# returaj/gan_mpc

Hardware: AMD Instinct MI355X
Metric: trajectories/sec (rollout+backward+critic step) at batch=1024, H=50 (higher is better)
Workload: dtype f32

## Files before the change

### gan_mpc_amd/csrc/gmpc_traj_rw.hip

```cpp
#include "gmpc_traj_layers.h"
#include "gmpc_ls_common.h"
#include "gmpc_launch.h"

#define GMPC_RW_THREADS 256
__host__ __device__ constexpr int rw_xk(int KH, int NHL) { return KH * NHL > 320 ? 64 : 0; }
__host__ __device__ constexpr int rw_khp(int KH) { return KH + 4; }
__host__ __device__ constexpr int rw_kb(int KH, int w) {
  return KH == 200 ? (w == 0 ? 0 : w == 1 ? 52 : w == 2 ? 104 : w == 3 ? 152 : 200) : (KH / 4) * w;
}

__host__ __device__ constexpr bool rw_row_in_lds(int k, int QX) { return (k >> 3) < QX && (k & 2) != 0; }
__host__ __device__ constexpr int rw_reg_index(int k, int QX) {
  int r = 0;
  for (int j = 0; j < k; ++j) r += rw_row_in_lds(j, QX) ? 0 : 1;
  return r;
}

__device__ __forceinline__ void rw_hidden_epilogue(f32x4_t d, int nn, int H, float4* hout, uint32_t* mbase,
                                                   size_t mstride, unsigned wbits) {
  const int lane = threadIdx.x & 63, wave = threadIdx.x >> 6;
  const bool valid = nn < H;
  const bool on0 = d[0] > 0.f && valid, on1 = d[1] > 0.f && valid;
  const bool on2 = d[2] > 0.f && valid, on3 = d[3] > 0.f && valid;
  const unsigned long long w0 = __ballot(on0), w1 = __ballot(on1), w2 = __ballot(on2), w3 = __ballot(on3);
  if (mbase != nullptr) {
    const unsigned long long word = lane == 0 ? w0 : lane == 1 ? w1 : lane == 2 ? w2 : w3;
    if (lane < 4 && ((wbits >> lane) & 1u)) {
      uint32_t* mp = mbase + (size_t)lane * mstride + 2 * wave;
      mp[0] = (uint32_t)word;
      mp[1] = (uint32_t)(word >> 32);
    }
  }
  if (valid) hout[nn] = make_float4(on0 ? d[0] : 0.f, on1 ? d[1] : 0.f, on2 ? d[2] : 0.f, on3 ? d[3] : 0.f);
}

template <int H, int XK>
__device__ __forceinline__ f32x4_t rw_layer(const float* wr, const float4* hin, const float4* wx, float bias) {
  static_assert(H % 8 == 0 && XK % 4 == 0 && 2 * XK <= H, "H");
  const int lane = threadIdx.x & 63;
  const float* hf = reinterpret_cast<const float*>(hin);
  constexpr int NR = (4 * H + 63) / 64;
  constexpr int QX = XK / 4;
  float ar[NR];
#pragma unroll
  for (int r = 0; r < NR; ++r) ar[r] = hf[64 * r + lane];
  constexpr int DX = 3;
  float4 xq[DX];
#pragma unroll
  for (int j = 0; j < DX; ++j)
    xq[j] = j < QX ? wx[j * GMPC_RW_THREADS + threadIdx.x] : make_float4(0.f, 0.f, 0.f, 0.f);
  f32x4_t d0 = {bias, bias, bias, bias}, d1 = {0.f, 0.f, 0.f, 0.f};
  __builtin_amdgcn_sched_barrier(0);
  rw_static_for<H / 8>([&](auto qc) __attribute__((always_inline)) {
    constexpr int q = decltype(qc)::value;
    const float4 x = xq[q % DX];
    if (q < QX && q + DX < QX) xq[q % DX] = wx[(q + DX) * GMPC_RW_THREADS + threadIdx.x];
    rw_static_for<8>([&](auto ec) __attribute__((always_inline)) {
      constexpr int e = decltype(ec)::value;
      constexpr int k = 8 * q + e;
      float w;
      if constexpr (rw_row_in_lds(k, QX)) w = e == 2 ? x.x : e == 3 ? x.y : e == 6 ? x.z : x.w;
      else { constexpr int ri = rw_reg_index(k, QX); w = wr[ri]; }
      if constexpr (e & 1) rw_mfma<k>(d1, ar[k >> 4], w);
      else rw_mfma<k>(d0, ar[k >> 4], w);
    });
    __builtin_amdgcn_sched_group_barrier(0x100, 1, 0);
    __builtin_amdgcn_sched_group_barrier(0x008, 8, 0);
  });
  return d0 + d1;
}

template <int K0, int K1, int KHP>
__device__ __forceinline__ f32x4_t rw_out_part(const float4* hin, const float* wlT, int n) {
  static_assert(K0 % 4 == 0 && K1 % 4 == 0 && K1 > K0, "float4 reads of the weight row");
  const int lane = threadIdx.x & 63;
  const float* hf = reinterpret_cast<const float*>(hin);
  constexpr int R0 = K0 >> 4, R1 = (K1 - 1) >> 4;
  float ar[R1 - R0 + 1];
#pragma unroll
  for (int r = R0; r <= R1; ++r) ar[r - R0] = hf[64 * r + lane];
  const float4* wrow = reinterpret_cast<const float4*>(wlT + (size_t)(lane < n ? lane : n - 1) * KHP + K0);
  float4 wv[(K1 - K0) / 4];
#pragma unroll
  for (int q = 0; q < (K1 - K0) / 4; ++q) wv[q] = wrow[q];
  f32x4_t d0 = {0.f, 0.f, 0.f, 0.f}, d1 = {0.f, 0.f, 0.f, 0.f};
  __builtin_amdgcn_sched_barrier(0);
  rw_static_for<(K1 - K0) / 4>([&](auto qc) __attribute__((always_inline)) {
    constexpr int q = decltype(qc)::value;
    constexpr int k = K0 + 4 * q;
    rw_mfma<k + 0>(d0, ar[((k + 0) >> 4) - R0], wv[q].x);
    rw_mfma<k + 1>(d1, ar[((k + 1) >> 4) - R0], wv[q].y);
    rw_mfma<k + 2>(d0, ar[((k + 2) >> 4) - R0], wv[q].z);
    rw_mfma<k + 3>(d1, ar[((k + 3) >> 4) - R0], wv[q].w);
  });
  return d0 + d1;
}

template <bool LS, int KH, int NHL, int K0Q>
__global__ __launch_bounds__(GMPC_RW_THREADS, 1) void k_traj_rw(TrajArgs a) {
  static_assert(KH % 16 == 0 || KH == 200, "output-layer K split in multiples of 4");
  constexpr int XK = rw_xk(KH, NHL), KHP = rw_khp(KH);
  extern __shared__ __attribute__((aligned(16))) char smem_traj[];
  float4* const actA = reinterpret_cast<float4*>(smem_traj);
  float4* const actB = actA + a.aw;
  float4* const part = actB + a.aw;
  float4* const ksp = part + a.pw;
  float4* const xcur = ksp + GMPC_THREADS;
  float* const wl_s = reinterpret_cast<float*>(xcur + 32);
  float4* const wx_s = reinterpret_cast<float4*>(wl_s + a.swl);
  __shared__ float s_alpha[GMPC_TB];
  __shared__ int s_bi[GMPC_TB], s_in[GMPC_TB];

  const int tid = threadIdx.x, wave = tid >> 6, lane = tid & 63;
  const int n = a.n, m = a.m, T = a.T;
  const int b0 = blockIdx.x * GMPC_TB;
  if (LS) {
    const int cnt = *a.nitems;
    if (b0 >= cnt || ls_round_form(cnt, a) != LS_FORM_RW) return;
    if (tid < GMPC_TB) ls_candidate(a, cnt, b0 + tid, &s_bi[tid], &s_in[tid], &s_alpha[tid]);
  } else if (tid < GMPC_TB) {
    s_bi[tid] = min(b0 + tid, a.B - 1);
    s_in[tid] = (b0 + tid) < a.B;
  }
  __syncthreads();
  float* const xf = reinterpret_cast<float*>(xcur);
  float* const aAf = reinterpret_cast<float*>(actA);
  const float* const pf = reinterpret_cast<const float*>(part);
  auto BI = [&](int c) -> int { return s_bi[c]; };
  auto INB = [&](int c) -> bool { return s_in[c] != 0; };
  auto CI = [&](int c) -> size_t { return (size_t)(b0 + c); };
  const int Lh = a.dyn.L - 1;
  const size_t mstride = (size_t)T * Lh * GMPC_MW;
  for (int e = tid; e < n * KHP; e += blockDim.x) {
    const int no = e / KHP, k = e - no * KHP;
    wl_s[e] = k < KH ? a.dyn.W[Lh][(size_t)k * n + no] : 0.f;
  }
  const float w0 = sigmoidf_(a.mpc_w[0]), w1 = sigmoidf_(a.mpc_w[1]), w2 = sigmoidf_(a.mpc_w[2]);

  const int nnA = 64 * wave + lane;
  float wr[NHL][KH];
  float w0r[4 * K0Q];
  float rbias[NHL + 1];
  {
#pragma unroll
    for (int k = 0; k < 4 * K0Q; ++k)
      w0r[k] = (k < n + m && nnA < KH) ? a.dyn.W[0][(size_t)k * KH + nnA] : 0.f;
    rw_static_for<NHL>([&](auto hc) __attribute__((always_inline)) {
      constexpr int hl = decltype(hc)::value;
      const float* Wl = a.dyn.W[hl + 1];
      constexpr int qx = hl == NHL - 1 ? XK / 4 : 0;
      rw_static_for<KH>([&](auto kc) __attribute__((always_inline)) {
        constexpr int k = decltype(kc)::value;
        if constexpr (!rw_row_in_lds(k, qx)) {
          constexpr int ri = rw_reg_index(k, qx);
          wr[hl][ri] = nnA < KH ? Wl[(size_t)k * KH + nnA] : 0.f;
        }
      });
      if constexpr (hl == NHL - 1) {
#pragma unroll 4
        for (int q = 0; q < XK / 4; ++q) {
          const float* wq = Wl + (size_t)(8 * q) * KH + nnA;
          wx_s[q * GMPC_RW_THREADS + tid] = nnA < KH ? make_float4(wq[2 * KH], wq[3 * KH], wq[6 * KH], wq[7 * KH])
                                                     : make_float4(0.f, 0.f, 0.f, 0.f);
        }
      }
    });
#pragma unroll
    for (int l = 0; l <= NHL; ++l) rbias[l] = nnA < KH ? a.dyn.b[l][nnA] : 0.f;
    for (int e = tid; e < 32; e += blockDim.x) xcur[e] = make_float4(0.f, 0.f, 0.f, 0.f);
    __syncthreads();
  }
  const float rbl = tid < 4 * n ? a.dyn.b[Lh][tid >> 2] : 0.f;
  auto put_u = [&](int c, int j, float u) { xf[(n + j) * 4 + c] = u; };

  unsigned wbits = 0;
#pragma unroll
  for (int c = 0; c < 4; ++c) wbits |= (INB(c) ? 1u : 0u) << c;
  for (int i = tid; i < n; i += blockDim.x) {
    const float* xs = LS ? a.X : a.x0;
    const size_t st = LS ? (size_t)(T + 1) * n : (size_t)n;
    float4 v = make_float4(xs[BI(0) * st + i], xs[BI(1) * st + i], xs[BI(2) * st + i], xs[BI(3) * st + i]);
    xcur[i] = v;
    if (!LS) {
#pragma unroll
      for (int c = 0; c < 4; ++c)
        if (INB(c)) a.X[(size_t)BI(c) * (T + 1) * n + i] = f4get(v, c);
    }
  }
  float objacc = 0.f;
  __syncthreads();
  TS_BEGIN();

  const bool rw_pf = GMPC_TB * m <= (int)(blockDim.x >> 3);
  const int rw_pp = tid >> 3, rw_l8 = tid & 7;
  const int rw_c = rw_pp / m, rw_j = rw_pp - rw_c * m;
  const bool rw_on = rw_pf && rw_pp < GMPC_TB * m;
  float pfK[4] = {0.f, 0.f, 0.f, 0.f}, pfX[4] = {0.f, 0.f, 0.f, 0.f}, pfk = 0.f, pfU = 0.f;
  auto rw_prefetch = [&](int t) {
    if (!rw_on) return;
    const int bc = BI(rw_c);
    const size_t ub = ((size_t)bc * T + t) * m + rw_j;
    if (LS) {
      const float* Kr = a.Kg + ub * n;
      const float* Xo = a.X + ((size_t)bc * (T + 1) + t) * n;
#pragma unroll
      for (int e = 0; e < 4; ++e) {
        const int i = rw_l8 + 8 * e;
        pfK[e] = i < n ? Kr[i] : 0.f;
        pfX[e] = i < n ? Xo[i] : 0.f;
      }
      pfk = a.kg[ub];
      pfU = a.Uio[ub];
    } else if (rw_l8 == 0) {
      pfU = a.U[ub];
    }
  };
  rw_prefetch(0);
  for (int t = 0; t < T; ++t) {
    if (rw_on) {
      float u = pfU;
      if (LS) {
        float du = 0.f;
#pragma unroll
        for (int e = 0; e < 4; ++e) {
          const int i = rw_l8 + 8 * e;
          if (i < n) du = fmaf(pfK[e], xf[i * 4 + rw_c] - pfX[e], du);
        }
        du += __shfl_xor(du, 4);
        du += __shfl_xor(du, 2);
        du += __shfl_xor(du, 1);
        u = pfU + fmaf(s_alpha[rw_c], pfk, du);
      }
      if (rw_l8 == 0) {
        if (LS && ((wbits >> rw_c) & 1u)) a.Uc[(CI(rw_c) * T + t) * m + rw_j] = u;
        put_u(rw_c, rw_j, u);
      }
    } else if (!rw_pf) {
      if (LS) {
        const int l16 = tid & 15;
        for (int p = tid >> 4; p < GMPC_TB * m; p += blockDim.x >> 4) {
          const int c = p / m, j = p - c * m;
          const int bc = BI(c);
          const size_t ub = ((size_t)bc * T + t) * m + j;
          const float* Kr = a.Kg + ub * n;
          const float* Xo = a.X + ((size_t)bc * (T + 1) + t) * n;
          float du = 0.f;
          for (int i = l16; i < n; i += 16) du = fmaf(Kr[i], xf[i * 4 + c] - Xo[i], du);
          du += __shfl_xor(du, 8);
          du += __shfl_xor(du, 4);
          du += __shfl_xor(du, 2);
          du += __shfl_xor(du, 1);
          if (l16 == 0) {
            const float u = a.Uio[ub] + fmaf(s_alpha[c], a.kg[ub], du);
            if ((wbits >> c) & 1u) a.Uc[(CI(c) * T + t) * m + j] = u;
            put_u(c, j, u);
          }
        }
      } else {
        for (int p = tid; p < GMPC_TB * m; p += blockDim.x) {
          const int c = p / m, j = p - c * m;
          put_u(c, j, a.U[((size_t)BI(c) * T + t) * m + j]);
        }
      }
    }
    if (t + 1 < T) rw_prefetch(t + 1);
    __syncthreads();
    TS_(0)
    uint32_t* mb = (LS ? a.maskc : a.masks) + (size_t)b0 * mstride + (size_t)t * Lh * GMPC_MW;
    {
      float ar[(K0Q + 3) / 4];
#pragma unroll
      for (int r = 0; r < (K0Q + 3) / 4; ++r) ar[r] = xf[64 * r + lane];
      f32x4_t d0 = {rbias[0], rbias[0], rbias[0], rbias[0]}, d1 = {0.f, 0.f, 0.f, 0.f};
      rw_static_for<2 * K0Q>([&](auto kc) __attribute__((always_inline)) {
        constexpr int k = 2 * decltype(kc)::value;
        rw_mfma<k>(d0, ar[k >> 4], w0r[k]);
        rw_mfma<k + 1>(d1, ar[(k + 1) >> 4], w0r[k + 1]);
      });
      rw_hidden_epilogue(d0 + d1, nnA, KH, actA, mb, mstride, wbits);
    }
    __syncthreads();
    TS_(2)
    float4* hin = actA;
    float4* hout = actB;
    rw_static_for<NHL>([&](auto hc) __attribute__((always_inline)) {
      constexpr int hl = decltype(hc)::value;
      const f32x4_t d = rw_layer<KH, (hl == NHL - 1 ? XK : 0)>(wr[hl], hin, wx_s, rbias[hl + 1]);
      rw_hidden_epilogue(d, nnA, KH, hout, mb + (hl + 1) * GMPC_MW, mstride, wbits);
      __syncthreads();
      TS_(3 + hl)
      float4* tmp = hin; hin = hout; hout = tmp;
    });
    {
      f32x4_t d;
      if (wave == 0) d = rw_out_part<rw_kb(KH, 0), rw_kb(KH, 1), KHP>(hin, wl_s, n);
      else if (wave == 1) d = rw_out_part<rw_kb(KH, 1), rw_kb(KH, 2), KHP>(hin, wl_s, n);
      else if (wave == 2) d = rw_out_part<rw_kb(KH, 2), rw_kb(KH, 3), KHP>(hin, wl_s, n);
      else d = rw_out_part<rw_kb(KH, 3), rw_kb(KH, 4), KHP>(hin, wl_s, n);
      if (lane < 32) part[wave * 32 + lane] = make_float4(d[0], d[1], d[2], d[3]);
    }
    __syncthreads();
    if (tid < 4 * n) {
      const int no = tid >> 2, c = tid & 3;
      float sum = pf[no * 4 + c];
#pragma unroll
      for (int w = 1; w < GMPC_RW_THREADS / 64; ++w) sum += pf[(w * 32 + no) * 4 + c];
      const float v = (sum + rbl) + xf[no * 4 + c];
      xf[no * 4 + c] = v;
      if ((wbits >> c) & 1u) {
        float* Xo = LS ? a.Xc : a.X;
        Xo[((LS ? CI(c) : (size_t)BI(c)) * (T + 1) + t + 1) * n + no] = v;
      }
    }
    if (LS) __syncthreads();
    TS_(6)
  }
#ifdef GMPC_TRAJ_STAMPS
  if (blockIdx.x == 0 && tid == 0)
    printf("k_traj_rw cycles per step: controls %llu L0 %llu L1 %llu L2 %llu out %llu\n", st_[0] / T, st_[2] / T,
           st_[3] / T, st_[4] / T, st_[6] / T);
#endif
  {
    __syncthreads();
    float* cs = aAf + wave * 64;
    const int c = wave;
    const int bc = BI(c);
    const float al = GMPC_ALPHA;
    for (int t0 = 0; t0 < T; t0 += 64) {
      const int t = t0 + lane;
      float cst = 0.f;
      if (t < T && INB(c)) {
        const float* xr = (LS && t > 0) ? a.Xc + (CI(c) * (T + 1) + t) * n
                                         : a.X + ((size_t)bc * (T + 1) + t) * n;
        const float* ur = LS ? a.Uc + (CI(c) * T + t) * m : a.U + ((size_t)bc * T + t) * m;
        const float* g = a.goal + ((size_t)bc * (T + 1) + t) * n;
        float dd = 0.f, uu = 0.f;
        for (int i = 0; i < n; ++i) {
          const float d = xr[i] - g[i];
          dd = fmaf(d, d, dd);
        }
        for (int j = 0; j < m; ++j) uu = fmaf(ur[j], ur[j], uu);
        cst = w0 * (sqrtf(uu + al * al) - al) + w1 * (sqrtf(dd + al * al) - al);
        if (!LS && a.costs) a.costs[(size_t)bc * (T + 1) + t] = cst;
      }
      cs[lane] = cst;
      __builtin_amdgcn_s_waitcnt(0xc07f);
      __builtin_amdgcn_wave_barrier();
      const int cnt = min(64, T - t0);
      for (int e = 0; e < cnt; ++e) objacc += cs[e];
      __builtin_amdgcn_wave_barrier();
    }
    __syncthreads();
  }
  {
    float4* in = xcur;
    float4* out = actA;
    const int Lc = a.cost.L - 1;
    for (int l = 0; l < Lc; ++l) {
      hidden_layer(a.cost.W[l], a.cost.b[l], a.cost.dims[l], a.cost.dims[l + 1], in, out, nullptr, 0,
                   0u, nullptr);
      __syncthreads();
      in = out;
      out = (out == actA) ? actB : actA;
    }
    const int fo = a.cost.dims[Lc + 1];
    dense_small<1>(a.cost.W[Lc], a.cost.dims[Lc], fo, in, part);
    const int c = wave & (GMPC_TB - 1);
    float yy = 0.f;
    for (int r = lane; r < fo; r += 64) {
      const float y = pf[r * 4 + c] + a.cost.b[Lc][r];
      yy = fmaf(y, y, yy);
    }
    yy = wave_sum(yy);
    const float cst = w2 * yy;
    objacc += cst;
    if (lane == 0 && wave < GMPC_TB) {
      if (!LS) {
        if (INB(c)) {
          if (a.costs) a.costs[(size_t)BI(c) * (T + 1) + T] = cst;
          a.obj[BI(c)] = objacc;
        }
      } else if (INB(c)) {
        a.objc[CI(c)] = objacc;
      }
    }
  }
}

static int rw_width(const TrajArgs& a) {
  const int Lh = a.dyn.L - 1;
  if (Lh != 3 || a.n > 32 || a.m > 32 || a.n + a.m > 32) return 0;
  const int H = a.dyn.dims[1];
  if (H != 200 && H != 128 && H != 64) return 0;
  for (int l = 1; l <= Lh; ++l)
    if (a.dyn.dims[l] != H) return 0;
  return H;
}
bool gmpc_traj_rw_shape(const TrajArgs& a) { return rw_width(a) != 0; }

size_t gmpc_traj_rw_lds(TrajArgs& a) {
  const int H = rw_width(a);
  a.aw = traj_aw(a.n, a.m, a.dyn, &a.cost);
  a.pw = GMPC_RW_THREADS;
  a.sw0 = 0;
  a.swl = a.n * rw_khp(H);
  return ((size_t)2 * a.aw + a.pw + GMPC_THREADS + 32) * sizeof(float4) +
         ((size_t)a.swl + (size_t)rw_xk(H, 2) * GMPC_RW_THREADS) * sizeof(float);
}

template <int KH, int K0Q>
static void launch_rw(const TrajArgs& a, bool ls, int grid, size_t lds, hipStream_t s) {
  static bool attr = false;
  if (!attr) {
    const void* ks[] = {reinterpret_cast<const void*>(&k_traj_rw<false, KH, 2, K0Q>),
                        reinterpret_cast<const void*>(&k_traj_rw<true, KH, 2, K0Q>)};
    for (const void* k : ks) {
      (void)hipFuncSetAttribute(k, hipFuncAttributeMaxDynamicSharedMemorySize, 128 * 1024);
      (void)hipGetLastError();
    }
    attr = true;
  }
  if (!ls) hipLaunchKernelGGL((k_traj_rw<false, KH, 2, K0Q>), dim3(grid), dim3(GMPC_RW_THREADS), lds, s, a);
  else hipLaunchKernelGGL((k_traj_rw<true, KH, 2, K0Q>), dim3(grid), dim3(GMPC_RW_THREADS), lds, s, a);
}

void gmpc_launch_traj_rw(const TrajArgs& a, bool ls, int grid, size_t lds, hipStream_t s) {
  const bool small = a.n + a.m <= 24;
  switch (rw_width(a)) {
    case 200:
      if (small) launch_rw<200, 6>(a, ls, grid, lds, s);
      else launch_rw<200, 8>(a, ls, grid, lds, s);
      break;
    case 128: launch_rw<128, 8>(a, ls, grid, lds, s); break;
    case 64: launch_rw<64, 8>(a, ls, grid, lds, s); break;
    default: break;
  }
}
```

Before: 834,800.

## Keep rollout state in registers and use buffer loads/stores in non-LS trajectory kernel

For the non-line-search rollout path, the layer-0 input vector (state plus control) is now kept in per-lane registers instead of being staged through LDS. This removes the control-staging phase and its barrier at each step. Controls for step t+2 are prefetched with raw buffer loads whose out-of-range offsets act as masks. State outputs and ReLU mask words are written with buffer stores (masks assembled via writelane), replacing the per-lane branching on validity. The change adds inline assembly and register pressure, and adds a T limit so the 32-bit buffer offsets stay in range.

After: 856,400, median of 6. +2.6%, better.

```diff
diff --git a/gan_mpc_amd/csrc/gmpc_traj_rw.hip b/gan_mpc_amd/csrc/gmpc_traj_rw.hip
--- a/gan_mpc_amd/csrc/gmpc_traj_rw.hip
+++ b/gan_mpc_amd/csrc/gmpc_traj_rw.hip
@@ -32,6 +32,37 @@
     }
   }
   if (valid) hout[nn] = make_float4(on0 ? d[0] : 0.f, on1 ? d[1] : 0.f, on2 ? d[2] : 0.f, on3 ? d[3] : 0.f);
+}
+
+#define GMPC_RW_OOB 0xFFFFFFF0u
+__device__ __forceinline__ __amdgpu_buffer_rsrc_t rw_rsrc(const void* p, size_t bytes) {
+  const unsigned long long v = reinterpret_cast<unsigned long long>(p);
+  const unsigned lo = __builtin_amdgcn_readfirstlane((unsigned)v), hi = __builtin_amdgcn_readfirstlane((unsigned)(v >> 32));
+  void* q = reinterpret_cast<void*>(((unsigned long long)hi << 32) | lo);
+  return __builtin_amdgcn_make_buffer_rsrc(q, 0, __builtin_amdgcn_readfirstlane((int)bytes), 0x00020000);
+}
+
+__device__ __forceinline__ void rw_writelanes(unsigned& lo, unsigned& hi, unsigned long long w0, unsigned long long w1,
+                                              unsigned long long w2) {
+  asm("s_nop 4\n\t"
+      "v_writelane_b32 %0, %2, 0\n\tv_writelane_b32 %1, %3, 0\n\t"
+      "v_writelane_b32 %0, %4, 1\n\tv_writelane_b32 %1, %5, 1\n\t"
+      "v_writelane_b32 %0, %6, 2\n\tv_writelane_b32 %1, %7, 2"
+      : "+v"(lo), "+v"(hi)
+      : "s"((unsigned)w0), "s"((unsigned)(w0 >> 32)), "s"((unsigned)w1), "s"((unsigned)(w1 >> 32)), "s"((unsigned)w2),
+        "s"((unsigned)(w2 >> 32)));
+}
+
+__device__ __forceinline__ void rw_hidden_epilogue_counted(f32x4_t d, int nn, int H, float4* hout,
+                                                           __amdgpu_buffer_rsrc_t rsm, unsigned moff, int soff) {
+  const bool on0 = d[0] > 0.f, on1 = d[1] > 0.f, on2 = d[2] > 0.f, on3 = d[3] > 0.f;
+  const unsigned long long w0 = __ballot(on0), w1 = __ballot(on1), w2 = __ballot(on2), w3 = __ballot(on3);
+  unsigned lo = (unsigned)w3, hi = (unsigned)(w3 >> 32);
+  rw_writelanes(lo, hi, w0, w1, w2);
+  typedef unsigned v2u_t __attribute__((ext_vector_type(2)));
+  const v2u_t wv = {lo, hi};
+  __builtin_amdgcn_raw_buffer_store_b64(wv, rsm, moff, soff, 0);
+  if (nn < H) hout[nn] = make_float4(on0 ? d[0] : 0.f, on1 ? d[1] : 0.f, on2 ? d[2] : 0.f, on3 ? d[3] : 0.f);
 }
 
 template <int H, int XK>
@@ -188,6 +219,36 @@
     }
   }
   float objacc = 0.f;
+
+  constexpr int NR0 = (K0Q + 3) / 4;
+  float ar0[NR0], pfu[NR0], blr[NR0];
+  unsigned uoff[NR0], xoff[NR0], moff = GMPC_RW_OOB;
+  bool isx[NR0];
+  __amdgpu_buffer_rsrc_t rsU, rsX, rsM;
+  if constexpr (!LS) {
+    const size_t nsl = min(GMPC_TB, a.B - b0);
+    rsU = rw_rsrc(a.U + (size_t)b0 * T * m, nsl * T * m * 4);
+    rsX = rw_rsrc(a.X + (size_t)b0 * (T + 1) * n, nsl * (T + 1) * n * 4);
+    rsM = rw_rsrc(a.masks + (size_t)b0 * mstride, nsl * mstride * 4);
+    const int c = lane & 3;
+    const bool wen = (wbits >> c) & 1u;
+    const int dc = BI(c) - b0;
+    if (lane < 4 && wen && a.masks != nullptr) moff = (unsigned)(((size_t)lane * mstride + 2 * wave) * 4);
+#pragma unroll
+    for (int r = 0; r < NR0; ++r) {
+      const int row = 16 * r + (lane >> 2);
+      isx[r] = row < n;
+      const bool isu = row >= n && row < n + m;
+      blr[r] = isx[r] ? a.dyn.b[Lh][row] : 0.f;
+      ar0[r] = isx[r] ? a.x0[(size_t)BI(c) * n + row] : 0.f;
+      uoff[r] = isu ? (unsigned)((dc * T * m + (row - n)) * 4) : GMPC_RW_OOB;
+      xoff[r] = (isx[r] && wen && wave == 0) ? (unsigned)((dc * (T + 1) * n + row) * 4) : GMPC_RW_OOB;
+      const float u0 = __uint_as_float(__builtin_amdgcn_raw_buffer_load_b32(rsU, uoff[r], 0, 0));
+      pfu[r] = __uint_as_float(__builtin_amdgcn_raw_buffer_load_b32(rsU, uoff[r], min(1, T - 1) * m * 4, 0));
+      if (!isx[r]) ar0[r] = u0;
+    }
+    __builtin_amdgcn_s_waitcnt(0x0f70);
+  }
   __syncthreads();
   TS_BEGIN();
 
@@ -200,26 +261,21 @@
     if (!rw_on) return;
     const int bc = BI(rw_c);
     const size_t ub = ((size_t)bc * T + t) * m + rw_j;
-    if (LS) {
-      const float* Kr = a.Kg + ub * n;
-      const float* Xo = a.X + ((size_t)bc * (T + 1) + t) * n;
-#pragma unroll
-      for (int e = 0; e < 4; ++e) {
-        const int i = rw_l8 + 8 * e;
-        pfK[e] = i < n ? Kr[i] : 0.f;
-        pfX[e] = i < n ? Xo[i] : 0.f;
-      }
-      pfk = a.kg[ub];
-      pfU = a.Uio[ub];
-    } else if (rw_l8 == 0) {
-      pfU = a.U[ub];
-    }
+    const float* Kr = a.Kg + ub * n;
+    const float* Xo = a.X + ((size_t)bc * (T + 1) + t) * n;
+#pragma unroll
+    for (int e = 0; e < 4; ++e) {
+      const int i = rw_l8 + 8 * e;
+      pfK[e] = i < n ? Kr[i] : 0.f;
+      pfX[e] = i < n ? Xo[i] : 0.f;
+    }
+    pfk = a.kg[ub];
+    pfU = a.Uio[ub];
   };
-  rw_prefetch(0);
+  if constexpr (LS) rw_prefetch(0);
   for (int t = 0; t < T; ++t) {
-    if (rw_on) {
-      float u = pfU;
-      if (LS) {
+    if constexpr (LS) {
+      if (rw_on) {
         float du = 0.f;
 #pragma unroll
         for (int e = 0; e < 4; ++e) {
@@ -229,14 +285,12 @@
         du += __shfl_xor(du, 4);
         du += __shfl_xor(du, 2);
         du += __shfl_xor(du, 1);
-        u = pfU + fmaf(s_alpha[rw_c], pfk, du);
-      }
-      if (rw_l8 == 0) {
-        if (LS && ((wbits >> rw_c) & 1u)) a.Uc[(CI(rw_c) * T + t) * m + rw_j] = u;
-        put_u(rw_c, rw_j, u);
-      }
-    } else if (!rw_pf) {
-      if (LS) {
+        const float u = pfU + fmaf(s_alpha[rw_c], pfk, du);
+        if (rw_l8 == 0) {
+          if ((wbits >> rw_c) & 1u) a.Uc[(CI(rw_c) * T + t) * m + rw_j] = u;
+          put_u(rw_c, rw_j, u);
+        }
+      } else if (!rw_pf) {
         const int l16 = tid & 15;
         for (int p = tid >> 4; p < GMPC_TB * m; p += blockDim.x >> 4) {
           const int c = p / m, j = p - c * m;
@@ -256,28 +310,25 @@
             put_u(c, j, u);
           }
         }
-      } else {
-        for (int p = tid; p < GMPC_TB * m; p += blockDim.x) {
-          const int c = p / m, j = p - c * m;
-          put_u(c, j, a.U[((size_t)BI(c) * T + t) * m + j]);
-        }
       }
-    }
-    if (t + 1 < T) rw_prefetch(t + 1);
-    __syncthreads();
-    TS_(0)
-    uint32_t* mb = (LS ? a.maskc : a.masks) + (size_t)b0 * mstride + (size_t)t * Lh * GMPC_MW;
+      if (t + 1 < T) rw_prefetch(t + 1);
+      __syncthreads();
+      TS_(0)
+    }
+    uint32_t* mb = a.maskc + (size_t)b0 * mstride + (size_t)t * Lh * GMPC_MW;
+    const int msoff = t * Lh * GMPC_MW * 4;
     {
-      float ar[(K0Q + 3) / 4];
-#pragma unroll
-      for (int r = 0; r < (K0Q + 3) / 4; ++r) ar[r] = xf[64 * r + lane];
+      float ar[NR0];
+#pragma unroll
+      for (int r = 0; r < NR0; ++r) ar[r] = LS ? xf[64 * r + lane] : ar0[r];
       f32x4_t d0 = {rbias[0], rbias[0], rbias[0], rbias[0]}, d1 = {0.f, 0.f, 0.f, 0.f};
       rw_static_for<2 * K0Q>([&](auto kc) __attribute__((always_inline)) {
         constexpr int k = 2 * decltype(kc)::value;
         rw_mfma<k>(d0, ar[k >> 4], w0r[k]);
         rw_mfma<k + 1>(d1, ar[(k + 1) >> 4], w0r[k + 1]);
       });
-      rw_hidden_epilogue(d0 + d1, nnA, KH, actA, mb, mstride, wbits);
+      if constexpr (LS) rw_hidden_epilogue(d0 + d1, nnA, KH, actA, mb, mstride, wbits);
+      else rw_hidden_epilogue_counted(d0 + d1, nnA, KH, actA, rsM, moff, msoff);
     }
     __syncthreads();
     TS_(2)
@@ -286,7 +337,8 @@
     rw_static_for<NHL>([&](auto hc) __attribute__((always_inline)) {
       constexpr int hl = decltype(hc)::value;
       const f32x4_t d = rw_layer<KH, (hl == NHL - 1 ? XK : 0)>(wr[hl], hin, wx_s, rbias[hl + 1]);
-      rw_hidden_epilogue(d, nnA, KH, hout, mb + (hl + 1) * GMPC_MW, mstride, wbits);
+      if constexpr (LS) rw_hidden_epilogue(d, nnA, KH, hout, mb + (hl + 1) * GMPC_MW, mstride, wbits);
+      else rw_hidden_epilogue_counted(d, nnA, KH, hout, rsM, moff, msoff + (hl + 1) * GMPC_MW * 4);
       __syncthreads();
       TS_(3 + hl)
       float4* tmp = hin; hin = hout; hout = tmp;
@@ -300,20 +352,44 @@
       if (lane < 32) part[wave * 32 + lane] = make_float4(d[0], d[1], d[2], d[3]);
     }
     __syncthreads();
-    if (tid < 4 * n) {
-      const int no = tid >> 2, c = tid & 3;
-      float sum = pf[no * 4 + c];
-#pragma unroll
-      for (int w = 1; w < GMPC_RW_THREADS / 64; ++w) sum += pf[(w * 32 + no) * 4 + c];
-      const float v = (sum + rbl) + xf[no * 4 + c];
-      xf[no * 4 + c] = v;
-      if ((wbits >> c) & 1u) {
-        float* Xo = LS ? a.Xc : a.X;
-        Xo[((LS ? CI(c) : (size_t)BI(c)) * (T + 1) + t + 1) * n + no] = v;
+    if constexpr (LS) {
+      if (tid < 4 * n) {
+        const int no = tid >> 2, c = tid & 3;
+        float sum = pf[no * 4 + c];
+#pragma unroll
+        for (int w = 1; w < GMPC_RW_THREADS / 64; ++w) sum += pf[(w * 32 + no) * 4 + c];
+        const float v = (sum + rbl) + xf[no * 4 + c];
+        xf[no * 4 + c] = v;
+        if ((wbits >> c) & 1u) a.Xc[(CI(c) * (T + 1) + t + 1) * n + no] = v;
       }
-    }
-    if (LS) __syncthreads();
+      __syncthreads();
+    } else {
+      const int tn = min(t + 2, T - 1);
+      float v[NR0];
+#pragma unroll
+      for (int r = 0; r < NR0; ++r) {
+        const int e = 64 * r + lane;
+        float sum = pf[e];
+#pragma unroll
+        for (int w = 1; w < GMPC_RW_THREADS / 64; ++w) sum += pf[w * 128 + e];
+        v[r] = (sum + blr[r]) + ar0[r];
+        ar0[r] = isx[r] ? v[r] : pfu[r];
+      }
+#pragma unroll
+      for (int r = 0; r < NR0; ++r)
+        pfu[r] = __uint_as_float(__builtin_amdgcn_raw_buffer_load_b32(rsU, uoff[r], tn * m * 4, 0));
+#pragma unroll
+      for (int r = 0; r < NR0; ++r)
+        __builtin_amdgcn_raw_buffer_store_b32(__float_as_uint(v[r]), rsX, xoff[r], (t + 1) * n * 4, 0);
+    }
     TS_(6)
+  }
+  if constexpr (!LS) {
+    if (wave == 0) {
+#pragma unroll
+      for (int r = 0; r < NR0; ++r)
+        if (isx[r]) xf[64 * r + lane] = ar0[r];
+    }
   }
 #ifdef GMPC_TRAJ_STAMPS
   if (blockIdx.x == 0 && tid == 0)
@@ -390,6 +466,7 @@
 static int rw_width(const TrajArgs& a) {
   const int Lh = a.dyn.L - 1;
   if (Lh != 3 || a.n > 32 || a.m > 32 || a.n + a.m > 32) return 0;
+  if (a.T > (1 << 20)) return 0;
   const int H = a.dyn.dims[1];
   if (H != 200 && H != 128 && H != 64) return 0;
   for (int l = 1; l <= Lh; ++l)
```
